# danping/CoSLAM

Measured on AMD Instinct MI355X. Metric: frames/sec for track+local-BA loop, 8 cams 640x480 x 2000 feats (one frame = all 8 cameras), higher is better.
Workload: dtype f32 (KLT, f16 pyramid storage) + f64 (pose, BA)

## Files before the change

### coslam_amd/csrc/poseupdate.hip

```cpp
#include <atomic>
#include <cstdlib>
#include <vector>

#include "cs_common.h"
#include "project_dev.h"
#include "history_view.h"
#include "register_rows_dev.h"
#include "small_ops.h"

#pragma clang fp contract(off)

namespace {

constexpr int PU_MAX_CAMS = 16;
constexpr int PU_MAX_HIST = 512;
constexpr int PU_MAX_STORE = 1 << 16;
constexpr int PU_LPS = 8;

struct PuArgs {
    int nCams, N, nMap, cam0, nCamsRun;
    int gateBlocks, dynBlocksPerCam;
    const int* pointFeat;
    const double* R;
    const double* t;
// ... 318 lines not shown
    }
    const unsigned long long b = __builtin_amdgcn_ballot_w64(fail);
    if (live && r == 0) {
        const bool anyFail = ((b >> (MG_LPC * g)) & ((1ull << MG_LPC) - 1ull)) != 0ull;
        A.out[(size_t)p * A.nCams + c] = s < 0 ? 255 : (cut ? 2 : (anyFail ? 0 : 1));
    }
}


struct MgCache {
    int slot1;
    int f1;
    int upto;
    int ok;
    double M[3];
    int epoch;
    int pad;
};
static_assert(sizeof(MgCache) == 48, "cs_register_mergability_cache_bytes");
struct MgRunCore {
    MgCore a;
    int W, count, curFrame;
    double tolPix;
    MgCache* cache;
    int epoch, fromMin;
    int* counts;
    const int* list;
    int nList;
    const int* flags;
};
struct MgRunArgs : MgRunCore {
    cs_poseupdate_cam cam[PU_MAX_CAMS];
};
constexpr int MG_GAP_MAX = 2 * MG_LPC;
struct MgMiss {
    int p, s, start, end;
};
template <int NT>
__device__ __forceinline__ void mg_running_rows(const MgRunCore& B, const cs_poseupdate_cam* cams, const int* list, int nList, int c, int bx,
                                                double* mg_pose, MgMiss* missList, int& nMiss) {
    const MgCore& A = B.a;
    const int tid = threadIdx.x, N = A.N, H = A.H, W = B.W;
    if (list && (int)(bx * (NT / MG_LPC)) < nList && list[bx * (NT / MG_LPC)] < 0) return;
    const cs_poseupdate_cam& C = cams[c];
    const double* hR = A.histR + (size_t)c * H * 9;
    const double* hT = A.histT + (size_t)c * H * 3;
    const double* hXY = A.histXY + (size_t)c * H * 2 * N;
    for (int q = tid; q < W * 12; q += NT) {
        const int j = q / 12, e = q - 12 * j, rs = (A.head - j + H) % H;
        mg_pose[q] = e < 9 ? hR[(size_t)rs * 9 + e] : hT[(size_t)rs * 3 + (e - 9)];
    }
    if (tid == 0) nMiss = 0;
    __syncthreads();
    const int lane = tid & 63, r = lane % MG_LPC, g = lane / MG_LPC;
    const unsigned long long gmask = ((1ull << MG_LPC) - 1ull) << (MG_LPC * g);
    const int jj = (bx * NT + tid) / MG_LPC;
    const int p = list ? (jj < nList ? list[jj] : -1) : (jj < A.P ? jj : -1);
    const bool live = p >= 0 && p < A.P;
    int s = live ? A.slot[(size_t)p * A.nCams + c] : -1;
    bool skipped = false;
    if (s >= 0 && B.flags && !(B.flags[(size_t)p * A.nCams + c] & 1)) skipped = true, s = -2;
    bool failW = false, cut = false, tailOK = true, hit = false, listed = false;
    int nTerms = 0;
    if (s >= 0) {
        double M[3], cov[9];
#pragma unroll
        for (int q = 0; q < 3; ++q) M[q] = A.M[3 * (size_t)p + q];
#pragma unroll
        for (int q = 0; q < 9; ++q) cov[q] = A.cov[9 * (size_t)p + q];
        const int f1 = C.trackSpan[s], f2 = C.trackSpan[N + s];
        const int len = f1 >= 0 ? f2 - f1 + 1 : 0;
        const int depth = len < W ? len : W;
        for (int j = r; j < depth && !failW; j += MG_LPC) {
            const double* R = mg_pose + 12 * j;
            const double* t = R + 9;
            const int rs = (A.head - j + H) % H;
            const double mx = hXY[(size_t)rs * 2 * N + s], my = hXY[(size_t)rs * 2 * N + N + s];
            failW = mg_term_fails(C.K, R, t, M, cov, A.sigma, mx, my);
        }
        failW = (__builtin_amdgcn_ballot_w64(failW) & gmask) != 0ull;
        const int end = B.curFrame - W;
        if (len > W) {
            MgCache* E = B.cache + (size_t)p * A.nCams + c;
            const MgCache e = *E;
            const PuProj q0 = pu_project(C.K, mg_pose, mg_pose + 9, M), q1 = pu_project(C.K, mg_pose, mg_pose + 9, e.M);
            const double du = q0.u / q0.w - q1.u / q1.w, dv = q0.v / q0.w - q1.v / q1.w;
            hit = e.slot1 == s + 1 && e.f1 == f1 && e.upto >= f1 - 1 && e.upto <= end && q0.w > 0 && q1.w > 0 &&
                  du * du + dv * dv <= B.tolPix * B.tolPix && (e.epoch == B.epoch || e.upto < B.fromMin);
            const int start = hit ? e.upto + 1 : f1;
            tailOK = hit ? e.ok != 0 : true;
            const bool shortGap = end - start + 1 <= MG_GAP_MAX;
            bool wrote = false;
            if (start > end) {
                wrote = hit;
            } else if (!tailOK) {
                wrote = true;
            } else if (B.curFrame - start >= B.count) {
                cut = !failW;
            } else if (shortGap && (hit || !failW)) {
                for (int f = start; f <= end && tailOK; f += MG_LPC) {
                    bool fail = false;
                    const int ff = f + r;
                    if (ff <= end) {
                        const int j = B.curFrame - ff, rs = ((A.head - j) % H + H) % H;
                        double Rt[12];
#pragma unroll
                        for (int q = 0; q < 9; ++q) Rt[q] = hR[(size_t)rs * 9 + q];
#pragma unroll
                        for (int q = 0; q < 3; ++q) Rt[9 + q] = hT[(size_t)rs * 3 + q];
                        const double mx = hXY[(size_t)rs * 2 * N + s], my = hXY[(size_t)rs * 2 * N + N + s];
                        fail = mg_term_fails(C.K, Rt, Rt + 9, M, cov, A.sigma, mx, my);
                        ++nTerms;
                    }
                    if (__builtin_amdgcn_ballot_w64(fail) & gmask) tailOK = false;
                }
                wrote = true;
            } else if (!failW) {
                listed = true;
                if (r == 0) {
                    const int k = atomicAdd(&nMiss, 1);
                    missList[k] = MgMiss{p, s, start, end};
                }
            }
            if (wrote && r == 0) {
                MgCache w;
                w.slot1 = s + 1, w.f1 = f1, w.upto = end, w.ok = tailOK ? 1 : 0;
                w.M[0] = hit ? e.M[0] : M[0], w.M[1] = hit ? e.M[1] : M[1], w.M[2] = hit ? e.M[2] : M[2], w.epoch = B.epoch, w.pad = 0;
                *E = w;
            }
        } else if (len > 0 && r == 0) {
            MgCache w;
            w.slot1 = s + 1, w.f1 = f1, w.upto = f1 - 1, w.ok = 1;
            w.M[0] = M[0], w.M[1] = M[1], w.M[2] = M[2], w.epoch = B.epoch, w.pad = 0;
            B.cache[(size_t)p * A.nCams + c] = w;
        }
    }
    if (live && r == 0 && !listed) A.out[(size_t)p * A.nCams + c] = s == -1 ? 255 : (skipped ? 0 : (cut ? 2 : (failW || !tailOK ? 0 : 1)));
    __syncthreads();
    const int wv = tid >> 6, nM = nMiss;
    for (int k = wv; k < nM; k += NT / 64) {
        const MgMiss m = missList[k];
        double M[3], cov[9];
#pragma unroll
        for (int q = 0; q < 3; ++q) M[q] = A.M[3 * (size_t)m.p + q];
#pragma unroll
        for (int q = 0; q < 9; ++q) cov[q] = A.cov[9 * (size_t)m.p + q];
        bool ok = true;
        for (int f = m.start; f <= m.end && ok; f += 64) {
            bool fail = false;
            const int ff = f + lane;
            if (ff <= m.end) {
                const int j = B.curFrame - ff, rs = ((A.head - j) % H + H) % H;
                double Rt[12];
#pragma unroll
                for (int q = 0; q < 9; ++q) Rt[q] = hR[(size_t)rs * 9 + q];
#pragma unroll
                for (int q = 0; q < 3; ++q) Rt[9 + q] = hT[(size_t)rs * 3 + q];
                const double mx = hXY[(size_t)rs * 2 * N + m.s], my = hXY[(size_t)rs * 2 * N + N + m.s];
                fail = mg_term_fails(C.K, Rt, Rt + 9, M, cov, A.sigma, mx, my);
                ++nTerms;
            }
            if (__builtin_amdgcn_ballot_w64(fail)) ok = false;
        }
        if (lane == 0) {
            MgCache* E = B.cache + (size_t)m.p * A.nCams + c;
            const bool fresh = m.start == C.trackSpan[m.s];
            MgCache w;
            w.slot1 = m.s + 1, w.f1 = C.trackSpan[m.s], w.upto = m.end, w.ok = ok ? 1 : 0;
            w.M[0] = fresh ? M[0] : E->M[0], w.M[1] = fresh ? M[1] : E->M[1], w.M[2] = fresh ? M[2] : E->M[2], w.epoch = B.epoch, w.pad = 0;
            *E = w;
            A.out[(size_t)m.p * A.nCams + c] = ok ? 1 : 0;
        }
    }
    if (B.counts) {
        const unsigned long long bh = __builtin_amdgcn_ballot_w64(hit && r == 0), bw = __builtin_amdgcn_ballot_w64(listed && !hit && r == 0),
                                 bc = __builtin_amdgcn_ballot_w64(cut && r == 0);
        int terms = nTerms;
#pragma unroll
        for (int o = 32; o > 0; o >>= 1) terms += __shfl_xor(terms, o, 64);
        if (lane == 0) {
            if (bh) atomicAdd(B.counts, __popcll(bh));
            if (bw) atomicAdd(B.counts + 1, __popcll(bw));
            if (bc) atomicAdd(B.counts + 2, __popcll(bc));
            if (terms) atomicAdd(B.counts + 3, terms);
        }
    }
}
__global__ __launch_bounds__(256) void k_register_mergability_running(MgRunArgs B) {
    extern __shared__ double mg_pose[];
    __shared__ MgMiss missList[256 / MG_LPC];
    __shared__ int nMiss;
    CS_POSE_STREAM_PRIO();
    mg_running_rows<256>(B, B.cam, B.list, B.nList, B.a.cam0 + blockIdx.y, blockIdx.x, mg_pose, missList, nMiss);
}


struct UpArgs {
    int nCams, N, nMap, H, head, nHist, firstKeyFrame;
    const int* pointFeat;
    const int* lastFrame;
    const unsigned char* isCurrent;
    const double* histXY;
    const double* histR;
    const double* histT;
    double* mapPts;
    double* mapCov;
    const unsigned char* mapFlags;
    double sigma;
    int* counts;
    const double* cen;
    int refine;
    const unsigned char* select;
    const int4* featRef;
    const unsigned char* refStatic;
    const int4* segPool;
    int segCap, curFrame, stored;
    cs_poseupdate_cam cam[PU_MAX_CAMS];
};
constexpr int UP_LPP = 64;

static_assert(UP_LPP == 64 && PU_MAX_CAMS <= UP_LPP, "the covariance tail broadcasts from lane = camera of the point's own wave");

struct UpNormalEq {
    double N[6], g[3];
};
__device__ __forceinline__ void up_add_view(UpNormalEq& E, const double* __restrict__ iK, const double* __restrict__ R,
// ... 1415 lines not shown
    }
    if (h->count < 1) {
        cs_set_error("cs_register_mergability_running_dev: the history holds no frame");
        return CS_ERR_INVALID;
    }
    if (d_list && nList < 0) {
        cs_set_error("cs_register_mergability_running_list_dev: nList < 0");
        return CS_ERR_INVALID;
    }
    const int rows = d_list ? nList : P;
    if (P == 0 || nCamsRun == 0 || rows == 0) return CS_OK;
    MgRunArgs B;
    memset(&B, 0, sizeof(B));
    B.list = d_list, B.nList = nList, B.flags = d_flags;
    MgCore& A = B.a;
    A.cam0 = cam0;
    A.nCams = h->nCams, A.N = h->N, A.P = P, A.H = h->H, A.head = h->head, A.nHist = hist_walk(h);
    A.sigma = pixelErrVar;
    A.M = d_M, A.cov = d_cov, A.slot = d_slot, A.out = d_mergeable;
    A.histXY = h->xy, A.histR = h->R, A.histT = h->t;
    for (int c = 0; c < h->nCams; ++c) {
        if (!cams[c].K || !cams[c].trackSpan) {
            cs_set_error("cs_register_mergability_running_dev: null pointer in camera %d", c);
            return CS_ERR_INVALID;
        }
        B.cam[c] = cams[c];
    }
    B.W = hist_walk(h), B.count = h->count, B.curFrame = h->lastFrame;
    B.epoch = h->tailEpoch, B.fromMin = h->tailFromMin;
    B.tolPix = tolPix;
    B.cache = (MgCache*)d_cache;
    B.counts = d_counts;
    CS_HIP(hipSetDevice(h->device));
    hipLaunchKernelGGL(k_register_mergability_running, dim3((rows * MG_LPC + 255) / 256, nCamsRun), dim3(256), sizeof(double) * 12 * (size_t)B.W,
                       (hipStream_t)hip_stream, B);
    CS_HIP(hipGetLastError());
    return CS_OK;
}

extern "C" int cs_track_history_set_poses_dev(cs_track_history* h, void* hip_stream, int n, const int* d_cam, const int* d_frame,
                                              const double* d_R, const double* d_t) {
    if (!h || n < 0 || (n > 0 && (!d_cam || !d_frame || !d_R || !d_t))) {
        cs_set_error("cs_track_history_set_poses_dev: bad arguments");
        return CS_ERR_INVALID;
    }
    if (n == 0 || h->count < 1) return CS_OK;
    h->ringVersion += 1;
    h->tailEpoch += 1, h->tailFromMin = -0x7fffffff;
    CS_HIP(hipSetDevice(h->device));
    hipLaunchKernelGGL(k_history_set_poses, dim3((n * 12 + 255) / 256), dim3(256), 0, (hipStream_t)hip_stream, n, d_cam, d_frame, d_R, d_t,
                       h->R, h->t, h->nCams, h->H, h->head, h->count, h->lastFrame);
    CS_HIP(hipGetLastError());
    return CS_OK;
}

namespace {
int hist_span(const char* who, cs_track_history* h, void* hip_stream, int set, int firstFrame, int nFrames, double* d_R, double* d_t) {
    if (!h || nFrames < 0 || (nFrames > 0 && (!d_R || !d_t))) {
        cs_set_error("%s: bad arguments", who);
        return CS_ERR_INVALID;
    }
    if (nFrames == 0) return CS_OK;
    if (firstFrame + nFrames - 1 > h->lastFrame || h->lastFrame - firstFrame >= h->count) {
        cs_set_error("%s: frames %d..%d are not all in the ring (it holds %d frame(s), the newest %d)", who, firstFrame, firstFrame + nFrames - 1,
                     h->count, h->lastFrame);
        return CS_ERR_INVALID;
    }
// ... 598 lines not shown
    int* lists;
    int* rvCounts;
    cs_register_pass pass;
    cs_register_cam rcam[RG_MAX_CAMS];
    MgRunCore mg;
    RvArgs rv;
    ArArgs ar;
};
static_assert(sizeof(RrArgs) <= 4096, "k_revisit_rounds: the arguments must fit the kernel-argument segment");
template <int MC>
__global__ __launch_bounds__(RR_THREADS) void k_revisit_rounds(RrArgs A) {
    extern __shared__ double rr_pose[];
    __shared__ MgMiss missList[RR_THREADS / MG_LPC];
    __shared__ int nMiss;
    __shared__ int sCnt[RR_THREADS / 64][5];
    if (rd_ld(A.rvCounts) == 0) return;
    CS_POSE_STREAM_PRIO();
    const int tid = threadIdx.x, lane = tid & 63, wave = tid >> 6, C = A.rv.nCams, cap = A.rv.cap, N = A.rv.N;
    const cs_register_pass& Q = A.pass;
    int cnt[5] = {0, 0, 0, 0, 0};
    for (int r = 0; r < A.nRounds; ++r) {
        const int listed = rd_ld(A.rvCounts + r);
        if (listed == 0) break;
        const int n = listed < cap ? listed : cap;
        const int* list = A.lists + (size_t)r * cap;
        for (int k = wave; k < n * C; k += RR_THREADS / 64) {
            const int row = k / C, c = k - row * C, p = list[row];
            if (p < 0) continue;
            const cs_register_cam& Cm = A.rcam[c];
            const size_t o = (size_t)p * C + c;
            int outSlot = -1, outFlags = 0;
            double m0 = 0, m1 = 0, var[4] = {0, 0, 0, 0}, ivar[4] = {0, 0, 0, 0}, outDist = 0;
            Proj q;
            if (rg_pair_begin(Q, Cm, o, p, A.W, A.H, q, m0, m1, var, ivar, outSlot)) {
                double dMin;
                int iMin;
                rg_pair_scan_wave(Cm, N, lane, m0, m1, ivar, dMin, iMin);
                rg_pair_finish(Q, Cm, p, N, q, m0, m1, dMin, iMin, outSlot, outFlags, outDist);
            }
            if (lane == 0) rg_pair_store(Q, o, outSlot, outFlags, outDist, m0, m1, var);
        }
        __syncthreads();
        const int nB = (n * MG_LPC + RR_THREADS - 1) / RR_THREADS;
        for (int c = 0; c < C; ++c)
            for (int bx = 0; bx < nB; ++bx) {
                mg_running_rows<RR_THREADS>(A.mg, A.ar.cam, list, cap, c, bx, rr_pose, missList, nMiss);
                __syncthreads();
            }
        {
            const bool more = r + 1 < A.nRounds;
            const RvRound Rd{list, A.rvCounts + r, more ? A.lists + (size_t)(r + 1) * cap : nullptr, more ? A.rvCounts + r + 1 : nullptr};
            if (n <= RR_THREADS) {
                rv_decide_rows<MC>(A.rv, Rd);
            } else {
                int* rowCode = (int*)(rr_pose + 12 * (size_t)A.mg.W);
                rv_decide_rows_looped<MC, RR_THREADS>(A.rv, Rd, n, rowCode, rowCode + MC * RV_MAX_ROWS);
            }
        }
        __syncthreads();
        for (int j = tid; j < n; j += RR_THREADS) {
            const int m = list[j];
            if (m >= 0 && m < A.ar.nMap && !A.ar.select[m]) fr_advance_row(A.ar.F, A.ar.cam, m, cnt);
        }
        __syncthreads();
        for (int j = wave; j < n; j += RR_THREADS / 64) {
            const int m = list[j];
            if (m >= 0 && m < A.ar.nMap && A.ar.select[m]) ar_refine_row(A.ar, m, lane, cnt);
        }
        __syncthreads();
    }
    if (A.ar.F.counts) {
#pragma unroll
        for (int k = 0; k < 5; ++k) {
            int v = cnt[k];
#pragma unroll
            for (int o = 32; o > 0; o >>= 1) v += __shfl_xor(v, o, 64);
            if (lane == 0) sCnt[wave][k] = v;
        }
        __syncthreads();
// ... 485 lines not shown
```

### coslam_amd/csrc/register.hip

```cpp
#include "cs_common.h"
#include "register_rows_dev.h"

#include <cfloat>

#pragma clang fp contract(off)

namespace {


struct RgArgs {
    int nCams, N, W, H, nPass, cam0;
    cs_register_pass pass[2];
    cs_register_cam cam[RG_MAX_CAMS];
};


constexpr int RG_WAVES = 8;
constexpr int RG_ROWS = RG_WAVES > 6 ? RG_WAVES : 6;
constexpr int RG_CHUNK = 512;

__global__ __launch_bounds__(64 * RG_WAVES) void k_register_search(RgArgs A) {
    extern __shared__ double lds[];
    CS_POSE_STREAM_PRIO();
    const int lane = threadIdx.x & 63, wave = threadIdx.x >> 6;
    const int c = A.cam0 + blockIdx.y;
    const cs_register_pass& Q = A.pass[blockIdx.z];
    const int j = blockIdx.x * 64 + lane;
    if (Q.list && (int)(blockIdx.x * 64) < Q.P && Q.list[blockIdx.x * 64] < 0) return;
    const int p = Q.list ? (j < Q.P ? Q.list[j] : -1) : (j < Q.P ? j : -1);
    const cs_register_cam& C = A.cam[c];
    const int N = A.N;
    const int CH = N < RG_CHUNK ? N : RG_CHUNK;
    double* sx = lds;
    double* sy = lds + CH;
    double* cd = lds + 2 * CH;
    int* ci = (int*)(cd + RG_ROWS * 64);
    const size_t o = (size_t)(p < 0 ? 0 : p) * A.nCams + c;
    int outSlot = -1, outFlags = 0;
    double m0 = 0, m1 = 0, var[4] = {0, 0, 0, 0}, outDist = 0;
    double ivar[4] = {0, 0, 0, 0};
    bool search = false;
    Proj q;
    if (wave == 0 && p >= 0) search = rg_pair_begin(Q, C, o, p, A.W, A.H, q, m0, m1, var, ivar, outSlot);
    if (__syncthreads_or(search)) {
        double* sq = cd;
        if (wave == 0) {
            sq[lane] = m0;
            sq[64 + lane] = m1;
#pragma unroll
            for (int k = 0; k < 4; ++k) sq[(2 + k) * 64 + lane] = ivar[k];
        }
        __syncthreads();
        if (wave != 0) {
            m0 = sq[lane];
            m1 = sq[64 + lane];
#pragma unroll
            for (int k = 0; k < 4; ++k) ivar[k] = sq[(2 + k) * 64 + lane];
        }
        const double* __restrict__ xs = C.xy;
        const double* __restrict__ ys = C.xy + N;
        const int* __restrict__ st = C.state;
        double dMin = DBL_MAX;
        int iMin = 0x7fffffff;
        for (int base = 0; base < N; base += CH) {
            const int n = (N - base) < CH ? (N - base) : CH;
            if (base) __syncthreads();
            for (int i = threadIdx.x; i < n; i += 64 * RG_WAVES) {
                const int s = st[base + i];
                const bool in = (s == 0 || s == 1);
                sx[i] = in ? xs[base + i] : __builtin_nan("");
                sy[i] = in ? ys[base + i] : __builtin_nan("");
            }
            __syncthreads();
            const int per = (n + RG_WAVES - 1) / RG_WAVES;
            const int lo = wave * per, hi = (lo + per) < n ? (lo + per) : n;
            for (int i = lo; i < hi; ++i) {
                const double d = maha_dist2(m0, m1, sx[i], sy[i], ivar);
                if (d < dMin) {
                    dMin = d;
                    iMin = base + i;
                }
            }
        }
        cd[wave * 64 + lane] = dMin;
        ci[wave * 64 + lane] = iMin;
        __syncthreads();
        if (wave == 0 && search) {
#pragma unroll 4
            for (int w = 1; w < RG_WAVES; ++w) {
                const double d2 = cd[w * 64 + lane];
                const int i2 = ci[w * 64 + lane];
                if (d2 < dMin || (d2 == dMin && i2 < iMin)) {
                    dMin = d2;
                    iMin = i2;
                }
            }
            rg_pair_finish(Q, C, p, N, q, m0, m1, dMin, iMin, outSlot, outFlags, outDist);
        }
    }
    if (wave == 0 && p >= 0) rg_pair_store(Q, o, outSlot, outFlags, outDist, m0, m1, var);
}

__global__ __launch_bounds__(1024) void k_register_list(int nCams, int nMap, const int* __restrict__ mapCount, const int* __restrict__ pointFeat,
                                                        const unsigned char* __restrict__ mapFlags, int* __restrict__ list,
                                                        int* __restrict__ listCount, int* __restrict__ slotTable, int listCap,
                                                        int* __restrict__ overflow) {
    __shared__ unsigned long long bits[1024];
    __shared__ int waveSum[16];
    const int tid = threadIdx.x, lane = tid & 63, wv = tid >> 6;
    const int live = mapCount ? (*mapCount < nMap ? *mapCount : nMap) : nMap;
    const bool vec4 = (nCams & 3) == 0 && (reinterpret_cast<uintptr_t>(pointFeat) & 15) == 0;
    const bool vec4s = (nCams & 3) == 0 && (reinterpret_cast<uintptr_t>(slotTable) & 15) == 0;
    const int oldCount = listCount ? (*listCount < nMap ? (*listCount < 0 ? 0 : *listCount) : nMap) : nMap;
    for (int w = tid; w < (nMap + 63) / 64; w += 1024) bits[w] = 0ull;
    __syncthreads();
// ... 127 lines not shown
        cs_set_error("cs_register_search_passes_dev: 1 or 2 passes");
        return CS_ERR_INVALID;
    }
    RgArgs A;
    memset(&A, 0, sizeof(A));
    A.nCams = nCams, A.N = N, A.W = W, A.H = H, A.nPass = nPass, A.cam0 = cam0;
    int maxP = 0;
    for (int k = 0; k < nPass; ++k) {
        const cs_register_pass& q = passes[k];
        int rc = check_args("cs_register_search_passes_dev", nCams, cams, N, W, H, q.P, q.sigmaSearch, q.maxDist, q.sigmaMerge);
        if (rc != CS_OK) return rc;
        if (q.P > 0 && (!q.M || !q.cov || !q.pointFeat || !q.slot || !q.m || !q.var || !q.dist || !q.flags)) {
            cs_set_error("cs_register_search_passes_dev: null pointer in pass %d", k);
            return CS_ERR_INVALID;
        }
        if (q.mapFlags && !(q.maxDistDynamic > 0)) {
            cs_set_error("cs_register_search_passes_dev: pass %d has mapFlags but maxDistDynamic <= 0", k);
            return CS_ERR_INVALID;
        }
        A.pass[k] = q;
        if (q.P > maxP) maxP = q.P;
    }
    if (maxP == 0 || nCamsRun == 0) return CS_OK;
    for (int c = cam0; c < cam0 + nCamsRun; ++c) {
        const cs_register_cam& q = cams[c];
        if (!q.K || !q.R || !q.t || !q.xy || !q.state || !q.slot2map) {
            cs_set_error("cs_register_search_passes_dev: null pointer in camera %d", c);
            return CS_ERR_INVALID;
        }
        A.cam[c] = q;
    }
    CS_HIP(hipSetDevice(device));
    const int CH = N < RG_CHUNK ? N : RG_CHUNK;
    const size_t ldsBytes = (size_t)2 * CH * sizeof(double) + (size_t)RG_ROWS * 64 * sizeof(double) + (size_t)RG_WAVES * 64 * sizeof(int);
    hipLaunchKernelGGL(k_register_search, dim3((unsigned)((maxP + 63) / 64), (unsigned)nCamsRun, (unsigned)nPass), dim3(64 * RG_WAVES), ldsBytes,
                       (hipStream_t)hip_stream, A);
    CS_CHECK_LAUNCH();
    return CS_OK;
}

extern "C" int cs_register_search_dev(int device, void* hip_stream, int nCams, const cs_register_cam* cams, int N, int W, int H,
                                      int P, const double* d_M, const double* d_cov, const int* d_pointFeat, double sigmaSearch,
                                      double maxDist, double sigmaMerge, int* d_slot, double* d_m, double* d_var, double* d_dist,
                                      int* d_flags) {
    int rc = check_args("cs_register_search_dev", nCams, cams, N, W, H, P, sigmaSearch, maxDist, sigmaMerge);
    if (rc != CS_OK) return rc;
    if (P == 0) return CS_OK;
    if (!d_M || !d_cov || !d_pointFeat || !d_slot || !d_m || !d_var || !d_dist || !d_flags) {
        cs_set_error("cs_register_search_dev: null pointer");
        return CS_ERR_INVALID;
    }
    cs_register_pass q;
    memset(&q, 0, sizeof(q));
    q.P = P, q.sigmaSearch = sigmaSearch, q.maxDist = maxDist, q.sigmaMerge = sigmaMerge;
    q.M = d_M, q.cov = d_cov, q.pointFeat = d_pointFeat, q.slot = d_slot, q.m = d_m, q.var = d_var, q.dist = d_dist, q.flags = d_flags;
    return cs_register_search_passes_dev(device, hip_stream, nCams, cams, N, W, H, 1, &q);
}

namespace {

struct RdArgs {
    int nCams, N, P, mapBase, nSweeps, onlyCam, kinds;
    const int* slot;
    const int* flags;
    const unsigned char* mergeable;
    const unsigned char* mapFlags;
    int* pointFeat;
// ... 606 lines not shown
```

### coslam_amd/csrc/register_rows_dev.h

```cpp
#pragma once

#include "cs_common.h"

#include <cfloat>

#pragma clang fp contract(off)

namespace {

constexpr int RG_MAX_CAMS = 16;

struct Proj {
    double u, v, w;
    double KR[9];
};

__device__ __forceinline__ void projection_cov(const Proj& q, const double* __restrict__ cov, double sigma, double var[4]) {
    const double ww = q.w * q.w;
    double J[6], JC[6];
#pragma unroll
    for (int j = 0; j < 3; ++j) {
        J[j] = (q.KR[j] * q.w - q.u * q.KR[6 + j]) / ww;
        J[3 + j] = (q.KR[3 + j] * q.w - q.v * q.KR[6 + j]) / ww;
    }
#pragma unroll
    for (int i = 0; i < 2; ++i)
#pragma unroll
        for (int j = 0; j < 3; ++j) JC[3 * i + j] = (J[3 * i] * cov[j] + J[3 * i + 1] * cov[3 + j]) + J[3 * i + 2] * cov[6 + j];
#pragma unroll
    for (int i = 0; i < 2; ++i)
#pragma unroll
        for (int j = 0; j < 2; ++j) {
            const double s = (JC[3 * i] * J[3 * j] + JC[3 * i + 1] * J[3 * j + 1]) + JC[3 * i + 2] * J[3 * j + 2];
            var[2 * i + j] = (i == j) ? s + sigma * sigma : s;
        }
}

__device__ __forceinline__ void mat22_inv(const double A[4], double iA[4]) {
    const double det = A[0] * A[3] - A[1] * A[2];
    iA[0] = A[3] / det;
    iA[1] = -A[1] / det;
    iA[2] = -A[2] / det;
    iA[3] = A[0] / det;
}

__device__ __forceinline__ double maha_dist2(double mx, double my, double bx, double by, const double ivar[4]) {
    const double dx = mx - bx, dy = my - by;
    return dx * (ivar[0] * dx + ivar[1] * dy) + dy * (ivar[2] * dx + ivar[3] * dy);
}

__device__ __forceinline__ bool rg_pair_begin(const cs_register_pass& Q, const cs_register_cam& C, size_t o, int p, int W, int H, Proj& q,
                                              double& m0, double& m1, double var[4], double ivar[4], int& outSlot) {
    if (Q.pointFeat[o] >= 0) return false;
    const double *K = C.K, *R = C.R, *t = C.t, *M = Q.M + 3 * (size_t)p;
    const double X = ((R[0] * M[0] + R[1] * M[1]) + R[2] * M[2]) + t[0];
    const double Y = ((R[3] * M[0] + R[4] * M[1]) + R[5] * M[2]) + t[1];
    const double Z = ((R[6] * M[0] + R[7] * M[1]) + R[8] * M[2]) + t[2];
    if (Z < 0.0) {
        outSlot = -2;
        return false;
    }
    q.u = (K[0] * X + K[1] * Y) + K[2] * Z;
    q.v = (K[3] * X + K[4] * Y) + K[5] * Z;
    q.w = (K[6] * X + K[7] * Y) + K[8] * Z;
    m0 = q.u / q.w;
    m1 = q.v / q.w;
    if (m0 < 0 || m0 >= (double)W || m1 < 0 || m1 >= (double)H) {
        outSlot = -3;
        return false;
    }
#pragma unroll
    for (int i = 0; i < 3; ++i)
#pragma unroll
        for (int j = 0; j < 3; ++j) q.KR[3 * i + j] = (K[3 * i] * R[j] + K[3 * i + 1] * R[3 + j]) + K[3 * i + 2] * R[6 + j];
    projection_cov(q, Q.cov + 9 * (size_t)p, Q.sigmaSearch, var);
    mat22_inv(var, ivar);
    const bool dynPt = Q.mapFlags && (Q.mapFlags[p] & (CS_MAP_DYNAMIC | CS_MAP_FALSE | CS_MAP_UNCERTAIN)) == CS_MAP_DYNAMIC;
    const double sc = 1 / (dynPt ? Q.maxDistDynamic : Q.maxDist);
#pragma unroll
    for (int k = 0; k < 4; ++k) ivar[k] = ivar[k] * sc;
    return true;
}
__device__ __forceinline__ void rg_pair_finish(const cs_register_pass& Q, const cs_register_cam& C, int p, int N, const Proj& q, double m0,
                                               double m1, double dMin, int iMin, int& outSlot, int& outFlags, double& outDist) {
    if (iMin == 0x7fffffff) {
        outSlot = -4;
        return;
    }
    outSlot = iMin;
    outDist = dMin;
    if (C.slot2map[iMin] < 0) outFlags |= 1;
    if (C.isDynamic ? C.isDynamic[iMin] != 0 : (C.isStatic && C.isStatic[iMin] == 0)) outFlags |= 2;
    double v2[4], iv[4];
    projection_cov(q, Q.cov + 9 * (size_t)p, Q.sigmaMerge, v2);
    mat22_inv(v2, iv);
    if (!(maha_dist2(m0, m1, C.xy[iMin], C.xy[N + iMin], iv) > 1.0)) outFlags |= 4;
}
__device__ __forceinline__ void rg_pair_store(const cs_register_pass& Q, size_t o, int outSlot, int outFlags, double outDist, double m0, double m1,
                                              const double var[4]) {
    Q.slot[o] = outSlot;
    Q.flags[o] = outFlags;
    Q.dist[o] = outDist;
    Q.m[2 * o] = m0;
    Q.m[2 * o + 1] = m1;
#pragma unroll
    for (int k = 0; k < 4; ++k) Q.var[4 * o + k] = var[k];
}
__device__ __forceinline__ void rg_pair_scan_wave(const cs_register_cam& C, int N, int lane, double m0, double m1, const double ivar[4],
                                                  double& dMin, int& iMin) {
    dMin = DBL_MAX, iMin = 0x7fffffff;
    const double* __restrict__ xs = C.xy;
    const double* __restrict__ ys = C.xy + N;
    const int* __restrict__ st = C.state;
    for (int i = lane; i < N; i += 64) {
        const int s = st[i];
        if (s == 0 || s == 1) {
            const double d = maha_dist2(m0, m1, xs[i], ys[i], ivar);
            if (d < dMin) dMin = d, iMin = i;
        }
    }
#pragma unroll
    for (int off = 32; off > 0; off >>= 1) {
        const double d2 = __shfl_xor(dMin, off, 64);
        const int i2 = __shfl_xor(iMin, off, 64);
        if (d2 < dMin || (d2 == dMin && i2 < iMin)) dMin = d2, iMin = i2;
    }
}

constexpr int RD_MAX_CAMS = 16;
// ... 355 lines not shown
```

Baseline: 2064.

## Prefetch per-row state and double-buffer candidate staging in register kernels

The mergability running kernel now issues every per-row global load up front, before the block barrier: cache entry, point, covariance, a window of history observations, and the staged poses plus K held in registers. Loads are pinned with empty asm and waited on with an explicit vmcnt wait. The in-window checks then read from registers and an LDS copy of K. The register search kernel double-buffers its LDS candidate chunks so the next chunk's global loads overlap the current scan, broadcasts camera pose via readlane, and batches the pair-begin/finish loads ahead of their use. The aim is to hide global memory latency, at the cost of more registers and LDS, and the code now targets gfx9 only.

```diff
diff --git a/coslam_amd/csrc/poseupdate.hip b/coslam_amd/csrc/poseupdate.hip
--- a/coslam_amd/csrc/poseupdate.hip
+++ b/coslam_amd/csrc/poseupdate.hip
@@ -374,12 +374,257 @@
 struct MgRunArgs : MgRunCore {
     cs_poseupdate_cam cam[PU_MAX_CAMS];
 };
+constexpr int MG_WINDOW_PREFETCH = 8;
 constexpr int MG_GAP_MAX = 2 * MG_LPC;
 struct MgMiss {
     int p, s, start, end;
 };
+__device__ __forceinline__ bool mg_gap_walk(const MgRunCore& B, const double* K, const double* hR, const double* hT, const double* hXY, int s,
+                                            int start, int end, const double* M, const double* cov, int r, unsigned long long gmask, int& nTerms) {
+    const MgCore& A = B.a;
+    const int N = A.N, H = A.H;
+    bool tailOK = true;
+    for (int f = start; f <= end && tailOK; f += MG_LPC) {
+        bool fail = false;
+        const int ff = f + r;
+        if (ff <= end) {
+            const int j = B.curFrame - ff, rs = ((A.head - j) % H + H) % H;
+            double Rt[12];
+#pragma unroll
+            for (int q = 0; q < 9; ++q) Rt[q] = hR[(size_t)rs * 9 + q];
+#pragma unroll
+            for (int q = 0; q < 3; ++q) Rt[9 + q] = hT[(size_t)rs * 3 + q];
+            const double mx = hXY[(size_t)rs * 2 * N + s], my = hXY[(size_t)rs * 2 * N + N + s];
+            fail = mg_term_fails(K, Rt, Rt + 9, M, cov, A.sigma, mx, my);
+            ++nTerms;
+        }
+        if (__builtin_amdgcn_ballot_w64(fail) & gmask) tailOK = false;
+    }
+    return tailOK;
+}
+__device__ __forceinline__ void mg_cache_write(MgCache* E, int s, int f1, int upto, bool ok, double m0, double m1, double m2, int epoch) {
+    MgCache w;
+    w.slot1 = s + 1, w.f1 = f1, w.upto = upto, w.ok = ok ? 1 : 0;
+    w.M[0] = m0, w.M[1] = m1, w.M[2] = m2, w.epoch = epoch, w.pad = 0;
+    *E = w;
+}
 template <int NT>
+__device__ __forceinline__ void mg_phase_b_and_counts(const MgRunCore& B, const cs_poseupdate_cam& C, const double* K, const double* hR,
+                                                      const double* hT, const double* hXY, int c, const MgMiss* missList, int nM, bool hit,
+                                                      bool listed, bool cut, int nTerms) {
+    const MgCore& A = B.a;
+    const int tid = threadIdx.x, N = A.N, H = A.H;
+    const int lane = tid & 63, r = lane % MG_LPC, wv = tid >> 6;
+    for (int k = wv; k < nM; k += NT / 64) {
+        const MgMiss m = missList[k];
+        double M[3], cov[9];
+#pragma unroll
+        for (int q = 0; q < 3; ++q) M[q] = A.M[3 * (size_t)m.p + q];
+#pragma unroll
+        for (int q = 0; q < 9; ++q) cov[q] = A.cov[9 * (size_t)m.p + q];
+        bool ok = true;
+        for (int f = m.start; f <= m.end && ok; f += 64) {
+            bool fail = false;
+            const int ff = f + lane;
+            if (ff <= m.end) {
+                const int j = B.curFrame - ff, rs = ((A.head - j) % H + H) % H;
+                double Rt[12];
+#pragma unroll
+                for (int q = 0; q < 9; ++q) Rt[q] = hR[(size_t)rs * 9 + q];
+#pragma unroll
+                for (int q = 0; q < 3; ++q) Rt[9 + q] = hT[(size_t)rs * 3 + q];
+                const double mx = hXY[(size_t)rs * 2 * N + m.s], my = hXY[(size_t)rs * 2 * N + N + m.s];
+                fail = mg_term_fails(K, Rt, Rt + 9, M, cov, A.sigma, mx, my);
+                ++nTerms;
+            }
+            if (__builtin_amdgcn_ballot_w64(fail)) ok = false;
+        }
+        if (lane == 0) {
+            MgCache* E = B.cache + (size_t)m.p * A.nCams + c;
+            const bool fresh = m.start == C.trackSpan[m.s];
+            MgCache w;
+            w.slot1 = m.s + 1, w.f1 = C.trackSpan[m.s], w.upto = m.end, w.ok = ok ? 1 : 0;
+            w.M[0] = fresh ? M[0] : E->M[0], w.M[1] = fresh ? M[1] : E->M[1], w.M[2] = fresh ? M[2] : E->M[2], w.epoch = B.epoch, w.pad = 0;
+            *E = w;
+            A.out[(size_t)m.p * A.nCams + c] = ok ? 1 : 0;
+        }
+    }
+    if (B.counts) {
+        const unsigned long long bh = __builtin_amdgcn_ballot_w64(hit && r == 0), bw = __builtin_amdgcn_ballot_w64(listed && !hit && r == 0),
+                                 bc = __builtin_amdgcn_ballot_w64(cut && r == 0);
+        int terms = nTerms;
+#pragma unroll
+        for (int o = 32; o > 0; o >>= 1) terms += __shfl_xor(terms, o, 64);
+        if (lane == 0) {
+            if (bh) atomicAdd(B.counts, __popcll(bh));
+            if (bw) atomicAdd(B.counts + 1, __popcll(bw));
+            if (bc) atomicAdd(B.counts + 2, __popcll(bc));
+            if (terms) atomicAdd(B.counts + 3, terms);
+        }
+    }
+}
+template <int NT, int PF>
 __device__ __forceinline__ void mg_running_rows(const MgRunCore& B, const cs_poseupdate_cam* cams, const int* list, int nList, int c, int bx,
+                                                double* mg_pose, MgMiss* missList, int& nMiss) {
+    const MgCore& A = B.a;
+    const int tid = threadIdx.x, N = A.N, H = A.H, W = B.W;
+    const int lane = tid & 63, r = lane % MG_LPC, g = lane / MG_LPC;
+    const unsigned long long gmask = ((1ull << MG_LPC) - 1ull) << (MG_LPC * g);
+    const int row0 = bx * (NT / MG_LPC), jj = (bx * NT + tid) / MG_LPC;
+    int p = jj < A.P ? jj : -1;
+    if (list && nList > 0) {
+        int l0 = list[row0 < nList ? row0 : nList - 1], lj = list[jj < nList ? jj : nList - 1];
+        rg_pin(l0), rg_pin(lj);
+        if (row0 < nList && l0 < 0) return;
+        p = jj < nList ? lj : -1;
+    } else if (list) {
+        p = -1;
+    }
+    const cs_poseupdate_cam& C = cams[c];
+    const double* hR = A.histR + (size_t)c * H * 9;
+    const double* hT = A.histT + (size_t)c * H * 3;
+    const double* hXY = A.histXY + (size_t)c * H * 2 * N;
+    const bool live = p >= 0 && p < A.P;
+    const size_t pc = (size_t)(live ? p : 0) * A.nCams + c;
+    MgCache* const E = B.cache + pc;
+    int s = -1, fl = 1;
+    MgCache e;
+    e.slot1 = 0, e.f1 = 0, e.upto = 0, e.ok = 0, e.M[0] = e.M[1] = e.M[2] = 0.0, e.epoch = 0, e.pad = 0;
+    double M[3] = {0, 0, 0}, cov[9] = {0, 0, 0, 0, 0, 0, 0, 0, 0};
+    if (live) {
+        s = A.slot[pc];
+        if (B.flags) fl = B.flags[pc];
+        e = *E;
+#pragma unroll
+        for (int q = 0; q < 3; ++q) M[q] = A.M[3 * (size_t)p + q];
+#pragma unroll
+        for (int q = 0; q < 9; ++q) cov[q] = A.cov[9 * (size_t)p + q];
+    }
+    const int nPose = 12 * (W + 1), nStage = nPose + 9;
+    const double* Ks = mg_pose + nPose;
+    auto staged = [&](int q) {
+        if (q >= nPose) return C.K[q - nPose];
+        const int j = q / 12, k = q - 12 * j, rs = ((A.head - j) % H + H) % H;
+        return k < 9 ? hR[(size_t)rs * 9 + k] : hT[(size_t)rs * 3 + (k - 9)];
+    };
+    double pv[4];
+#pragma unroll
+    for (int u = 0; u < 4; ++u) {
+        const int q = tid + u * NT;
+        pv[u] = 0.0;
+        if (q < nStage) pv[u] = staged(q);
+    }
+    bool skipped = false;
+    if (s >= 0 && !(fl & 1)) skipped = true, s = -2;
+    int f1 = -1, f2 = -1;
+    double wx[PF], wy[PF], tx = 0.0, ty = 0.0;
+#pragma unroll
+    for (int u = 0; u < PF; ++u) wx[u] = wy[u] = 0.0;
+    if (s >= 0) {
+        f1 = C.trackSpan[s], f2 = C.trackSpan[N + s];
+#pragma unroll
+        for (int u = 0; u < PF; ++u) {
+            const int j = r + MG_LPC * u;
+            if (j < W) {
+                const int rs = (A.head - j + H) % H;
+                wx[u] = hXY[(size_t)rs * 2 * N + s], wy[u] = hXY[(size_t)rs * 2 * N + N + s];
+            }
+        }
+        const int rs = ((A.head - W) % H + H) % H;
+        tx = hXY[(size_t)rs * 2 * N + s], ty = hXY[(size_t)rs * 2 * N + N + s];
+    }
+#pragma unroll
+    for (int u = 0; u < 4; ++u)
+        if (tid + u * NT < nStage) mg_pose[tid + u * NT] = pv[u];
+    for (int q = tid + 4 * NT; q < nStage; q += NT) mg_pose[q] = staged(q);
+    if (tid == 0) nMiss = 0;
+    rg_pin(e.slot1), rg_pin(e.f1), rg_pin(e.upto), rg_pin(e.ok), rg_pin(e.epoch), rg_pin(f1), rg_pin(f2), rg_pin(tx), rg_pin(ty);
+#pragma unroll
+    for (int q = 0; q < 3; ++q) rg_pin(M[q]), rg_pin(e.M[q]);
+#pragma unroll
+    for (int q = 0; q < 9; ++q) rg_pin(cov[q]);
+#pragma unroll
+    for (int u = 0; u < PF; ++u) rg_pin(wx[u]), rg_pin(wy[u]);
+    rg_loads_arrived();
+    __syncthreads();
+    bool failW = false, cut = false, tailOK = true, hit = false, listed = false;
+    int nTerms = 0;
+    if (s >= 0) {
+        const int len = f1 >= 0 ? f2 - f1 + 1 : 0;
+        const int depth = len < W ? len : W;
+        const int end = B.curFrame - W;
+        int start = f1;
+        if (len > W) {
+            const PuProj q0 = pu_project(Ks, mg_pose, mg_pose + 9, M), q1 = pu_project(Ks, mg_pose, mg_pose + 9, e.M);
+            const double du = q0.u / q0.w - q1.u / q1.w, dv = q0.v / q0.w - q1.v / q1.w;
+            hit = e.slot1 == s + 1 && e.f1 == f1 && e.upto >= f1 - 1 && e.upto <= end && q0.w > 0 && q1.w > 0 &&
+                  du * du + dv * dv <= B.tolPix * B.tolPix && (e.epoch == B.epoch || e.upto < B.fromMin);
+            start = hit ? e.upto + 1 : f1;
+            tailOK = hit ? e.ok != 0 : true;
+        }
+        if (tailOK) {
+            for (int u0 = 0; r + MG_LPC * u0 < depth && !failW; u0 += PF) {
+                if (u0 > 0) {
+#pragma unroll
+                    for (int u = 0; u < PF; ++u) {
+                        const int j = r + MG_LPC * (u0 + u);
+                        if (j < depth) {
+                            const int rs = (A.head - j + H) % H;
+                            wx[u] = hXY[(size_t)rs * 2 * N + s], wy[u] = hXY[(size_t)rs * 2 * N + N + s];
+                        }
+                    }
+                }
+#pragma unroll 1
+                for (int u = 0; u < PF; ++u) {
+                    const int j = r + MG_LPC * (u0 + u);
+                    if (j >= depth || failW) break;
+                    const double* R = mg_pose + 12 * j;
+                    failW = mg_term_fails(Ks, R, R + 9, M, cov, A.sigma, wx[0], wy[0]);
+#pragma unroll
+                    for (int k = 0; k + 1 < PF; ++k) wx[k] = wx[k + 1], wy[k] = wy[k + 1];
+                }
+            }
+            failW = (__builtin_amdgcn_ballot_w64(failW) & gmask) != 0ull;
+        }
+        if (len > W) {
+            const bool shortGap = end - start + 1 <= MG_GAP_MAX;
+            bool wrote = false;
+            if (start > end) {
+                wrote = hit;
+            } else if (!tailOK) {
+                wrote = true;
+            } else if (B.curFrame - start >= B.count) {
+                cut = !failW;
+            } else if (shortGap && (hit || !failW)) {
+                if (start == end) {
+                    bool fail = false;
+                    if (r == 0) {
+                        fail = mg_term_fails(Ks, mg_pose + 12 * W, mg_pose + 12 * W + 9, M, cov, A.sigma, tx, ty);
+                        ++nTerms;
+                    }
+                    if (__builtin_amdgcn_ballot_w64(fail) & gmask) tailOK = false;
+                } else {
+                    tailOK = mg_gap_walk(B, Ks, hR, hT, hXY, s, start, end, M, cov, r, gmask, nTerms);
+                }
+                wrote = true;
+            } else if (!failW) {
+                listed = true;
+                if (r == 0) {
+                    const int k = atomicAdd(&nMiss, 1);
+                    missList[k] = MgMiss{p, s, start, end};
+                }
+            }
+            if (wrote && r == 0) mg_cache_write(E, s, f1, end, tailOK, hit ? e.M[0] : M[0], hit ? e.M[1] : M[1], hit ? e.M[2] : M[2], B.epoch);
+        } else if (len > 0 && r == 0) {
+            mg_cache_write(E, s, f1, f1 - 1, true, M[0], M[1], M[2], B.epoch);
+        }
+    }
+    if (live && r == 0 && !listed) A.out[(size_t)p * A.nCams + c] = s == -1 ? 255 : (skipped ? 0 : (cut ? 2 : (failW || !tailOK ? 0 : 1)));
+    __syncthreads();
+    mg_phase_b_and_counts<NT>(B, C, Ks, hR, hT, hXY, c, missList, nMiss, hit, listed, cut, nTerms);
+}
+template <int NT>
+__device__ __forceinline__ void mg_running_rows_serial(const MgRunCore& B, const cs_poseupdate_cam* cams, const int* list, int nList, int c, int bx,
                                                 double* mg_pose, MgMiss* missList, int& nMiss) {
     const MgCore& A = B.a;
     const int tid = threadIdx.x, N = A.N, H = A.H, W = B.W;
@@ -440,22 +685,7 @@
             } else if (B.curFrame - start >= B.count) {
                 cut = !failW;
             } else if (shortGap && (hit || !failW)) {
-                for (int f = start; f <= end && tailOK; f += MG_LPC) {
-                    bool fail = false;
-                    const int ff = f + r;
-                    if (ff <= end) {
-                        const int j = B.curFrame - ff, rs = ((A.head - j) % H + H) % H;
-                        double Rt[12];
-#pragma unroll
-                        for (int q = 0; q < 9; ++q) Rt[q] = hR[(size_t)rs * 9 + q];
-#pragma unroll
-                        for (int q = 0; q < 3; ++q) Rt[9 + q] = hT[(size_t)rs * 3 + q];
-                        const double mx = hXY[(size_t)rs * 2 * N + s], my = hXY[(size_t)rs * 2 * N + N + s];
-                        fail = mg_term_fails(C.K, Rt, Rt + 9, M, cov, A.sigma, mx, my);
-                        ++nTerms;
-                    }
-                    if (__builtin_amdgcn_ballot_w64(fail) & gmask) tailOK = false;
-                }
+                tailOK = mg_gap_walk(B, C.K, hR, hT, hXY, s, start, end, M, cov, r, gmask, nTerms);
                 wrote = true;
             } else if (!failW) {
                 listed = true;
@@ -464,76 +694,21 @@
                     missList[k] = MgMiss{p, s, start, end};
                 }
             }
-            if (wrote && r == 0) {
-                MgCache w;
-                w.slot1 = s + 1, w.f1 = f1, w.upto = end, w.ok = tailOK ? 1 : 0;
-                w.M[0] = hit ? e.M[0] : M[0], w.M[1] = hit ? e.M[1] : M[1], w.M[2] = hit ? e.M[2] : M[2], w.epoch = B.epoch, w.pad = 0;
-                *E = w;
-            }
+            if (wrote && r == 0) mg_cache_write(E, s, f1, end, tailOK, hit ? e.M[0] : M[0], hit ? e.M[1] : M[1], hit ? e.M[2] : M[2], B.epoch);
         } else if (len > 0 && r == 0) {
-            MgCache w;
-            w.slot1 = s + 1, w.f1 = f1, w.upto = f1 - 1, w.ok = 1;
-            w.M[0] = M[0], w.M[1] = M[1], w.M[2] = M[2], w.epoch = B.epoch, w.pad = 0;
-            B.cache[(size_t)p * A.nCams + c] = w;
+            mg_cache_write(B.cache + (size_t)p * A.nCams + c, s, f1, f1 - 1, true, M[0], M[1], M[2], B.epoch);
         }
     }
     if (live && r == 0 && !listed) A.out[(size_t)p * A.nCams + c] = s == -1 ? 255 : (skipped ? 0 : (cut ? 2 : (failW || !tailOK ? 0 : 1)));
     __syncthreads();
-    const int wv = tid >> 6, nM = nMiss;
-    for (int k = wv; k < nM; k += NT / 64) {
-        const MgMiss m = missList[k];
-        double M[3], cov[9];
-#pragma unroll
-        for (int q = 0; q < 3; ++q) M[q] = A.M[3 * (size_t)m.p + q];
-#pragma unroll
-        for (int q = 0; q < 9; ++q) cov[q] = A.cov[9 * (size_t)m.p + q];
-        bool ok = true;
-        for (int f = m.start; f <= m.end && ok; f += 64) {
-            bool fail = false;
-            const int ff = f + lane;
-            if (ff <= m.end) {
-                const int j = B.curFrame - ff, rs = ((A.head - j) % H + H) % H;
-                double Rt[12];
-#pragma unroll
-                for (int q = 0; q < 9; ++q) Rt[q] = hR[(size_t)rs * 9 + q];
-#pragma unroll
-                for (int q = 0; q < 3; ++q) Rt[9 + q] = hT[(size_t)rs * 3 + q];
-                const double mx = hXY[(size_t)rs * 2 * N + m.s], my = hXY[(size_t)rs * 2 * N + N + m.s];
-                fail = mg_term_fails(C.K, Rt, Rt + 9, M, cov, A.sigma, mx, my);
-                ++nTerms;
-            }
-            if (__builtin_amdgcn_ballot_w64(fail)) ok = false;
-        }
-        if (lane == 0) {
-            MgCache* E = B.cache + (size_t)m.p * A.nCams + c;
-            const bool fresh = m.start == C.trackSpan[m.s];
-            MgCache w;
-            w.slot1 = m.s + 1, w.f1 = C.trackSpan[m.s], w.upto = m.end, w.ok = ok ? 1 : 0;
-            w.M[0] = fresh ? M[0] : E->M[0], w.M[1] = fresh ? M[1] : E->M[1], w.M[2] = fresh ? M[2] : E->M[2], w.epoch = B.epoch, w.pad = 0;
-            *E = w;
-            A.out[(size_t)m.p * A.nCams + c] = ok ? 1 : 0;
-        }
-    }
-    if (B.counts) {
-        const unsigned long long bh = __builtin_amdgcn_ballot_w64(hit && r == 0), bw = __builtin_amdgcn_ballot_w64(listed && !hit && r == 0),
-                                 bc = __builtin_amdgcn_ballot_w64(cut && r == 0);
-        int terms = nTerms;
-#pragma unroll
-        for (int o = 32; o > 0; o >>= 1) terms += __shfl_xor(terms, o, 64);
-        if (lane == 0) {
-            if (bh) atomicAdd(B.counts, __popcll(bh));
-            if (bw) atomicAdd(B.counts + 1, __popcll(bw));
-            if (bc) atomicAdd(B.counts + 2, __popcll(bc));
-            if (terms) atomicAdd(B.counts + 3, terms);
-        }
-    }
+    mg_phase_b_and_counts<NT>(B, C, C.K, hR, hT, hXY, c, missList, nMiss, hit, listed, cut, nTerms);
 }
 __global__ __launch_bounds__(256) void k_register_mergability_running(MgRunArgs B) {
     extern __shared__ double mg_pose[];
     __shared__ MgMiss missList[256 / MG_LPC];
     __shared__ int nMiss;
     CS_POSE_STREAM_PRIO();
-    mg_running_rows<256>(B, B.cam, B.list, B.nList, B.a.cam0 + blockIdx.y, blockIdx.x, mg_pose, missList, nMiss);
+    mg_running_rows<256, MG_WINDOW_PREFETCH>(B, B.cam, B.list, B.nList, B.a.cam0 + blockIdx.y, blockIdx.x, mg_pose, missList, nMiss);
 }
 
 
@@ -2015,7 +2190,7 @@
     B.cache = (MgCache*)d_cache;
     B.counts = d_counts;
     CS_HIP(hipSetDevice(h->device));
-    hipLaunchKernelGGL(k_register_mergability_running, dim3((rows * MG_LPC + 255) / 256, nCamsRun), dim3(256), sizeof(double) * 12 * (size_t)B.W,
+    hipLaunchKernelGGL(k_register_mergability_running, dim3((rows * MG_LPC + 255) / 256, nCamsRun), dim3(256), sizeof(double) * 12 * (size_t)(B.W + 2),
                        (hipStream_t)hip_stream, B);
     CS_HIP(hipGetLastError());
     return CS_OK;
@@ -2680,7 +2855,8 @@
             int outSlot = -1, outFlags = 0;
             double m0 = 0, m1 = 0, var[4] = {0, 0, 0, 0}, ivar[4] = {0, 0, 0, 0}, outDist = 0;
             Proj q;
-            if (rg_pair_begin(Q, Cm, o, p, A.W, A.H, q, m0, m1, var, ivar, outSlot)) {
+            const RgCamPose Cp = rg_cam_pose(Cm, lane);
+            if (rg_pair_begin(Q, Cp, o, p, A.W, A.H, q, m0, m1, var, ivar, outSlot)) {
                 double dMin;
                 int iMin;
                 rg_pair_scan_wave(Cm, N, lane, m0, m1, ivar, dMin, iMin);
@@ -2692,7 +2868,7 @@
         const int nB = (n * MG_LPC + RR_THREADS - 1) / RR_THREADS;
         for (int c = 0; c < C; ++c)
             for (int bx = 0; bx < nB; ++bx) {
-                mg_running_rows<RR_THREADS>(A.mg, A.ar.cam, list, cap, c, bx, rr_pose, missList, nMiss);
+                mg_running_rows_serial<RR_THREADS>(A.mg, A.ar.cam, list, cap, c, bx, rr_pose, missList, nMiss);
                 __syncthreads();
             }
         {
diff --git a/coslam_amd/csrc/register.hip b/coslam_amd/csrc/register.hip
--- a/coslam_amd/csrc/register.hip
+++ b/coslam_amd/csrc/register.hip
@@ -18,22 +18,46 @@
 constexpr int RG_WAVES = 8;
 constexpr int RG_ROWS = RG_WAVES > 6 ? RG_WAVES : 6;
 constexpr int RG_CHUNK = 512;
+static_assert(RG_CHUNK == 64 * RG_WAVES, "k_register_search stages one slot of a chunk per thread");
+
+struct RgStaged {
+    int s;
+    double x, y;
+};
+__device__ __forceinline__ RgStaged rg_stage_load(const int* __restrict__ st, const double* __restrict__ xs, const double* __restrict__ ys, int n,
+                                                  unsigned i) {
+    RgStaged g{-1, 0.0, 0.0};
+    if ((int)i < n) g.s = st[i], g.x = xs[i], g.y = ys[i];
+    return g;
+}
+__device__ __forceinline__ void rg_stage_store(const RgStaged& g, double* sx, double* sy, int n, int i) {
+    if (i >= n) return;
+    const bool in = (g.s == 0 || g.s == 1);
+    sx[i] = in ? g.x : __builtin_nan("");
+    sy[i] = in ? g.y : __builtin_nan("");
+}
 
 __global__ __launch_bounds__(64 * RG_WAVES) void k_register_search(RgArgs A) {
     extern __shared__ double lds[];
     CS_POSE_STREAM_PRIO();
-    const int lane = threadIdx.x & 63, wave = threadIdx.x >> 6;
+    const int tid = threadIdx.x, lane = tid & 63, wave = tid >> 6;
     const int c = A.cam0 + blockIdx.y;
     const cs_register_pass& Q = A.pass[blockIdx.z];
-    const int j = blockIdx.x * 64 + lane;
-    if (Q.list && (int)(blockIdx.x * 64) < Q.P && Q.list[blockIdx.x * 64] < 0) return;
-    const int p = Q.list ? (j < Q.P ? Q.list[j] : -1) : (j < Q.P ? j : -1);
     const cs_register_cam& C = A.cam[c];
     const int N = A.N;
     const int CH = N < RG_CHUNK ? N : RG_CHUNK;
-    double* sx = lds;
-    double* sy = lds + CH;
-    double* cd = lds + 2 * CH;
+    const double* __restrict__ xs = C.xy;
+    const double* __restrict__ ys = C.xy + N;
+    const int* __restrict__ st = C.state;
+    const int j = blockIdx.x * 64 + lane;
+    int p = j < Q.P ? j : -1;
+    if (Q.list && j < Q.P) p = Q.list[j];
+    RgStaged g = rg_stage_load(st, xs, ys, CH, tid);
+    RgCamPose cam;
+    if (wave == 0) cam = rg_cam_pose(C, lane);
+    if (__builtin_amdgcn_readfirstlane(p) < 0) return;
+    double* stage = lds;
+    double* cd = lds + (N > CH ? 4 : 2) * CH;
     int* ci = (int*)(cd + RG_ROWS * 64);
     const size_t o = (size_t)(p < 0 ? 0 : p) * A.nCams + c;
     int outSlot = -1, outFlags = 0;
@@ -41,37 +65,29 @@
     double ivar[4] = {0, 0, 0, 0};
     bool search = false;
     Proj q;
-    if (wave == 0 && p >= 0) search = rg_pair_begin(Q, C, o, p, A.W, A.H, q, m0, m1, var, ivar, outSlot);
+    if (wave == 0) {
+        if (p >= 0) search = rg_pair_begin(Q, cam, o, p, A.W, A.H, q, m0, m1, var, ivar, outSlot);
+        cd[lane] = m0;
+        cd[64 + lane] = m1;
+#pragma unroll
+        for (int k = 0; k < 4; ++k) cd[(2 + k) * 64 + lane] = ivar[k];
+    }
+    rg_stage_store(g, stage, stage + CH, CH, tid);
     if (__syncthreads_or(search)) {
-        double* sq = cd;
-        if (wave == 0) {
-            sq[lane] = m0;
-            sq[64 + lane] = m1;
-#pragma unroll
-            for (int k = 0; k < 4; ++k) sq[(2 + k) * 64 + lane] = ivar[k];
-        }
-        __syncthreads();
         if (wave != 0) {
-            m0 = sq[lane];
-            m1 = sq[64 + lane];
-#pragma unroll
-            for (int k = 0; k < 4; ++k) ivar[k] = sq[(2 + k) * 64 + lane];
-        }
-        const double* __restrict__ xs = C.xy;
-        const double* __restrict__ ys = C.xy + N;
-        const int* __restrict__ st = C.state;
+            m0 = cd[lane];
+            m1 = cd[64 + lane];
+#pragma unroll
+            for (int k = 0; k < 4; ++k) ivar[k] = cd[(2 + k) * 64 + lane];
+        }
         double dMin = DBL_MAX;
         int iMin = 0x7fffffff;
-        for (int base = 0; base < N; base += CH) {
+        for (int base = 0, b = 0; base < N; base += CH, b ^= 1) {
             const int n = (N - base) < CH ? (N - base) : CH;
-            if (base) __syncthreads();
-            for (int i = threadIdx.x; i < n; i += 64 * RG_WAVES) {
-                const int s = st[base + i];
-                const bool in = (s == 0 || s == 1);
-                sx[i] = in ? xs[base + i] : __builtin_nan("");
-                sy[i] = in ? ys[base + i] : __builtin_nan("");
-            }
-            __syncthreads();
+            const int nb = base + CH, nn = (N - nb) < CH ? (N - nb) : CH;
+            if (nn > 0) g = rg_stage_load(st + nb, xs + nb, ys + nb, nn, tid);
+            const double* sx = stage + b * 2 * CH;
+            const double* sy = sx + CH;
             const int per = (n + RG_WAVES - 1) / RG_WAVES;
             const int lo = wave * per, hi = (lo + per) < n ? (lo + per) : n;
             for (int i = lo; i < hi; ++i) {
@@ -81,6 +97,8 @@
                     iMin = base + i;
                 }
             }
+            if (nn > 0) rg_stage_store(g, stage + (b ^ 1) * 2 * CH, stage + (b ^ 1) * 2 * CH + CH, nn, tid);
+            __syncthreads();
         }
         cd[wave * 64 + lane] = dMin;
         ci[wave * 64 + lane] = iMin;
@@ -274,7 +292,7 @@
     }
     CS_HIP(hipSetDevice(device));
     const int CH = N < RG_CHUNK ? N : RG_CHUNK;
-    const size_t ldsBytes = (size_t)2 * CH * sizeof(double) + (size_t)RG_ROWS * 64 * sizeof(double) + (size_t)RG_WAVES * 64 * sizeof(int);
+    const size_t ldsBytes = (size_t)(N > CH ? 4 : 2) * CH * sizeof(double) + (size_t)RG_ROWS * 64 * sizeof(double) + (size_t)RG_WAVES * 64 * sizeof(int);
     hipLaunchKernelGGL(k_register_search, dim3((unsigned)((maxP + 63) / 64), (unsigned)nCamsRun, (unsigned)nPass), dim3(64 * RG_WAVES), ldsBytes,
                        (hipStream_t)hip_stream, A);
     CS_CHECK_LAUNCH();
diff --git a/coslam_amd/csrc/register_rows_dev.h b/coslam_amd/csrc/register_rows_dev.h
--- a/coslam_amd/csrc/register_rows_dev.h
+++ b/coslam_amd/csrc/register_rows_dev.h
@@ -49,10 +49,40 @@
     return dx * (ivar[0] * dx + ivar[1] * dy) + dy * (ivar[2] * dx + ivar[3] * dy);
 }
 
-__device__ __forceinline__ bool rg_pair_begin(const cs_register_pass& Q, const cs_register_cam& C, size_t o, int p, int W, int H, Proj& q,
-                                              double& m0, double& m1, double var[4], double ivar[4], int& outSlot) {
-    if (Q.pointFeat[o] >= 0) return false;
-    const double *K = C.K, *R = C.R, *t = C.t, *M = Q.M + 3 * (size_t)p;
+struct RgCamPose {
+    double K[9], R[9], t[3];
+};
+__device__ __forceinline__ double rg_lane_value(double v, int l) {
+    return __hiloint2double(__builtin_amdgcn_readlane(__double2hiint(v), l), __builtin_amdgcn_readlane(__double2loint(v), l));
+}
+__device__ __forceinline__ RgCamPose rg_cam_pose(const cs_register_cam& C, int lane) {
+    const double* w = lane < 9 ? C.K + lane : (lane < 18 ? C.R + (lane - 9) : C.t + (lane < 21 ? lane - 18 : 0));
+    const double v = *w;
+    RgCamPose P;
+#pragma unroll
+    for (int i = 0; i < 9; ++i) P.K[i] = rg_lane_value(v, i), P.R[i] = rg_lane_value(v, 9 + i);
+#pragma unroll
+    for (int i = 0; i < 3; ++i) P.t[i] = rg_lane_value(v, 18 + i);
+    return P;
+}
+#if defined(__HIP_DEVICE_COMPILE__) && !defined(__GFX9__)
+#error "rg_loads_arrived: 0x0f70 is vmcnt(0), expcnt and lgkmcnt untouched, in the gfx9 family's s_waitcnt layout only"
+#endif
+__device__ __forceinline__ void rg_loads_arrived() { __builtin_amdgcn_s_waitcnt(0x0f70); }
+__device__ __forceinline__ void rg_pin(double& v) { asm volatile("" : "+v"(v)); }
+__device__ __forceinline__ void rg_pin(int& v) { asm volatile("" : "+v"(v)); }
+__device__ __forceinline__ bool rg_pair_begin(const cs_register_pass& Q, const RgCamPose& C, size_t o, int p, int W, int H, Proj& q, double& m0,
+                                              double& m1, double var[4], double ivar[4], int& outSlot) {
+    const int pf = Q.pointFeat[o];
+    const double *K = C.K, *R = C.R, *t = C.t;
+    double M[3], cov[9];
+#pragma unroll
+    for (int i = 0; i < 3; ++i) M[i] = Q.M[3 * (size_t)p + i];
+#pragma unroll
+    for (int i = 0; i < 9; ++i) cov[i] = Q.cov[9 * (size_t)p + i];
+    const unsigned char mf = Q.mapFlags ? Q.mapFlags[p] : 0;
+    rg_loads_arrived();
+    if (pf >= 0) return false;
     const double X = ((R[0] * M[0] + R[1] * M[1]) + R[2] * M[2]) + t[0];
     const double Y = ((R[3] * M[0] + R[4] * M[1]) + R[5] * M[2]) + t[1];
     const double Z = ((R[6] * M[0] + R[7] * M[1]) + R[8] * M[2]) + t[2];
@@ -73,9 +103,9 @@
     for (int i = 0; i < 3; ++i)
 #pragma unroll
         for (int j = 0; j < 3; ++j) q.KR[3 * i + j] = (K[3 * i] * R[j] + K[3 * i + 1] * R[3 + j]) + K[3 * i + 2] * R[6 + j];
-    projection_cov(q, Q.cov + 9 * (size_t)p, Q.sigmaSearch, var);
+    projection_cov(q, cov, Q.sigmaSearch, var);
     mat22_inv(var, ivar);
-    const bool dynPt = Q.mapFlags && (Q.mapFlags[p] & (CS_MAP_DYNAMIC | CS_MAP_FALSE | CS_MAP_UNCERTAIN)) == CS_MAP_DYNAMIC;
+    const bool dynPt = (mf & (CS_MAP_DYNAMIC | CS_MAP_FALSE | CS_MAP_UNCERTAIN)) == CS_MAP_DYNAMIC;
     const double sc = 1 / (dynPt ? Q.maxDistDynamic : Q.maxDist);
 #pragma unroll
     for (int k = 0; k < 4; ++k) ivar[k] = ivar[k] * sc;
@@ -87,14 +117,23 @@
         outSlot = -4;
         return;
     }
+    const int owner = C.slot2map[iMin];
+    const unsigned char* type = C.isDynamic ? C.isDynamic : C.isStatic;
+    unsigned char tv = 0;
+    if (type) tv = type[iMin];
+    const double fx = C.xy[iMin], fy = C.xy[N + iMin];
+    double cov[9];
+#pragma unroll
+    for (int i = 0; i < 9; ++i) cov[i] = Q.cov[9 * (size_t)p + i];
+    const bool dyn = C.isDynamic ? tv != 0 : (C.isStatic && tv == 0);
     outSlot = iMin;
     outDist = dMin;
-    if (C.slot2map[iMin] < 0) outFlags |= 1;
-    if (C.isDynamic ? C.isDynamic[iMin] != 0 : (C.isStatic && C.isStatic[iMin] == 0)) outFlags |= 2;
+    if (owner < 0) outFlags |= 1;
+    if (dyn) outFlags |= 2;
     double v2[4], iv[4];
-    projection_cov(q, Q.cov + 9 * (size_t)p, Q.sigmaMerge, v2);
+    projection_cov(q, cov, Q.sigmaMerge, v2);
     mat22_inv(v2, iv);
-    if (!(maha_dist2(m0, m1, C.xy[iMin], C.xy[N + iMin], iv) > 1.0)) outFlags |= 4;
+    if (!(maha_dist2(m0, m1, fx, fy, iv) > 1.0)) outFlags |= 4;
 }
 __device__ __forceinline__ void rg_pair_store(const cs_register_pass& Q, size_t o, int outSlot, int outFlags, double outDist, double m0, double m1,
                                               const double var[4]) {
```

Result: no change. 2060 (-0.2%).
